# AlejandroSilvestri/os1

Hardware: AMD Instinct MI355X
Metric: frames/sec extract+match, 1920x1080 @ 2000 ORB feats (higher is better)
Workload: dtype u8

## Files before the change

### include/orbfe.h

```cpp
#ifndef ORBFE_H_
#define ORBFE_H_

#include <stddef.h>
#include <stdint.h>

#ifdef __cplusplus
extern "C" {
#endif

#define ORBFE_OK 0
#define ORBFE_ERR_INVALID (-1)
#define ORBFE_ERR_NO_DEVICE (-2)
#define ORBFE_ERR_HIP (-3)
#define ORBFE_ERR_TOO_SMALL (-4)
#define ORBFE_ERR_OVERFLOW (-5)
#define ORBFE_ERR_UNSUPPORTED (-6)

typedef struct OrbfeKeyPoint {
  float x, y;
  float size;
  float angle;
  float response;
  int32_t octave;
  int32_t class_id;
// ... 44 lines not shown

int orbfe_extract(orbfe_extractor* h, const uint8_t* gray, int rows, int cols, size_t stride_bytes,
                  OrbfeKeyPoint* kps, uint8_t* desc, int cap, int* n_out);

int orbfe_extract_batch(orbfe_extractor* h, int nframes, const uint8_t* const* gray, int in_device_memory,
                        int rows, int cols, size_t stride_bytes, OrbfeKeyPoint* kps, uint8_t* desc, int cap,
                        int* n_out);

int orbfe_extract_batch_submit(orbfe_extractor* h, int nframes, const uint8_t* const* gray, int in_device_memory,
                               int rows, int cols, size_t stride_bytes);
int orbfe_extract_batch_collect(orbfe_extractor* h, OrbfeKeyPoint* kps, uint8_t* desc, int cap, int* n_out);
int orbfe_extract_batch_wait(orbfe_extractor* h);

typedef struct orbfe_sfi_chain orbfe_sfi_chain;
int orbfe_sfi_chain_create(const orbfe_extractor* h, orbfe_sfi_chain** out);
void orbfe_sfi_chain_destroy(orbfe_sfi_chain* c);
int orbfe_sfi_chain_set_isolated(orbfe_sfi_chain* c, int isolated);
int orbfe_sfi_chain_restart(orbfe_sfi_chain* c);
int orbfe_extract_batch_submit_matched(orbfe_extractor* h, orbfe_sfi_chain* chain, int nframes, const uint8_t* const* gray,
                                       int in_device_memory, int rows, int cols, size_t stride_bytes, const float bounds[4],
                                       int window_size, float nnratio, int check_orientation);
int orbfe_extract_batch_collect_matched(orbfe_extractor* h, OrbfeKeyPoint* kps, uint8_t* desc, int cap, int* n_out,
                                        int32_t* matches12, int* nmatches);

int orbfe_extractor_set_camera(orbfe_extractor* h, int camera_mode, float fx, float fy, float cx, float cy, const float* dist,
                               int ndist);
int orbfe_extractor_undistort(orbfe_extractor* h, float* xy, int n);

int orbfe_extractor_set_camera_equidistant(orbfe_extractor* h, float fx, float fy, float cx, float cy);
int orbfe_extractor_undistort_verdict(orbfe_extractor* h, const float* xy, int n, float* out, uint8_t* undecided);
int orbfe_extractor_equidistant_stats(const orbfe_extractor* h, long long stats[3]);
int orbfe_extract_undistorted(orbfe_extractor* h, const uint8_t* gray, int rows, int cols, size_t stride_bytes, OrbfeKeyPoint* kps,
                              uint8_t* desc, int cap, int* n_out, float* xy_un);
int orbfe_extract_batch_collect_undistorted(orbfe_extractor* h, OrbfeKeyPoint* kps, uint8_t* desc, int cap, int* n_out, float* xy_un,
                                            int32_t* matches12, int* nmatches);

int orbfe_debug_level_size(const orbfe_extractor* h, int level, int* w, int* hgt);
int orbfe_debug_level_copy(orbfe_extractor* h, int frame, int level, uint8_t* out );
int orbfe_debug_candidates(orbfe_extractor* h, int frame, int level, int32_t* xys, int cap, int* n_out);
int orbfe_debug_stage_ms(const orbfe_extractor* h, float out[5]);
int orbfe_debug_kernel_ms(orbfe_extractor* h, double out_ms[5], long long* batches, long long* frames, int reset);
int orbfe_debug_set_profiling(orbfe_extractor* h, int enable);
int orbfe_debug_fast_stamps(orbfe_extractor* h, unsigned long long out[8], int reset);
int orbfe_debug_sfi_records(orbfe_extractor* h, int32_t* out, int cap_records, int* n_out, int reset);
int orbfe_debug_sincos(orbfe_extractor* h, const float* angle_deg, int n, float* cos_out, float* sin_out);

int orbfe_debug_quadtree(const int16_t* x, const int16_t* y, const uint8_t* score, int n, int min_x, int max_x,
                         int min_y, int max_y, int n_target, int32_t* out_idx, int cap, int* n_out);
int orbfe_debug_sincos_host_check(uint32_t lo_bits, uint32_t hi_bits, uint32_t step, long long* mismatches);
int orbfe_debug_logf(orbfe_matcher* m, const float* x, int n, float* out);
int orbfe_debug_logf_host_check(uint32_t lo_bits, uint32_t hi_bits, uint32_t step, long long* mismatches);

typedef struct orbfe_stream orbfe_stream;
int orbfe_stream_create(int nfeatures, float scaleFactor, int nlevels, int iniThFAST, int minThFAST, int device_id,
                        int batch, int depth, orbfe_stream** out);
void orbfe_stream_destroy(orbfe_stream* s);
int orbfe_stream_set_matching(orbfe_stream* s, const float bounds[4], int window_size, float nnratio,
                              int check_orientation);
int orbfe_stream_set_isolated_batches(orbfe_stream* s, int isolated);
int orbfe_stream_batches_in_flight(const orbfe_stream* s);
int orbfe_stream_pop_hold(orbfe_stream* s, const OrbfeKeyPoint** kps, const uint8_t** desc, const int** n_kps, const int32_t** matches12,
                          const int** nmatches, int* ticket);
int orbfe_stream_release(orbfe_stream* s, int ticket);
int orbfe_stream_set_input_format(orbfe_stream* s, int format, int gray_variant);
int orbfe_stream_set_blur_variant(orbfe_stream* s, int variant);
int orbfe_stream_set_vocabulary(orbfe_stream* s, orbfe_vocabulary* v, int levelsup);
int orbfe_stream_bow_raw(orbfe_stream* s, int frame, const uint32_t** leaf_node, const uint32_t** level_node, int* n);
int orbfe_stream_set_camera(orbfe_stream* s, int camera_mode, float fx, float fy, float cx, float cy, const float* dist, int ndist);
int orbfe_stream_set_camera_equidistant(orbfe_stream* s, float fx, float fy, float cx, float cy);
int orbfe_stream_equidistant_stats(orbfe_stream* s, long long stats[3]);
int orbfe_stream_xy_un(orbfe_stream* s, const float** xy_un);
int orbfe_stream_capacity(const orbfe_stream* s);
int orbfe_stream_set_queue_slots(orbfe_stream* s, int nslots);
int orbfe_stream_queue_slots(const orbfe_stream* s);
int orbfe_stream_push(orbfe_stream* s, const uint8_t* const* gray, int in_device_memory, int rows, int cols,
                      size_t stride_bytes);
int orbfe_stream_pop(orbfe_stream* s, const OrbfeKeyPoint** kps, const uint8_t** desc, const int** n_kps,
                     const int32_t** matches12, const int** nmatches);
int orbfe_stream_stats(orbfe_stream* s, double out[4], int reset);
int orbfe_stream_kernel_ms(orbfe_stream* s, double out_ms[5], long long* batches, long long* frames, int reset);


int orbfe_hamming(const uint8_t a[32], const uint8_t b[32]);

int orbfe_matcher_create(int device_id, orbfe_matcher** out);
void orbfe_matcher_destroy(orbfe_matcher* m);
int orbfe_matcher_device(const orbfe_matcher* m);
int orbfe_matcher_upload_async(orbfe_matcher* m, void* dst_device, const void* src_host, size_t bytes);
int orbfe_matcher_synchronize(orbfe_matcher* m);

int orbfe_search_for_initialization(orbfe_matcher* m, const OrbfeKeyPoint* kps1, const uint8_t* desc1, int n1,
                                    const OrbfeKeyPoint* kps2, const uint8_t* desc2, int n2,
                                    const float bounds[4], float* prev_xy, int32_t* matches12, int window_size,
                                    float nnratio, int check_orientation, int* nmatches);

int orbfe_search_for_initialization_batch(orbfe_matcher* m, int npairs, const OrbfeKeyPoint* const* kps1,
                                          const uint8_t* const* desc1, const int* n1,
                                          const OrbfeKeyPoint* const* kps2, const uint8_t* const* desc2,
                                          const int* n2, const float bounds[4], float* const* prev_xy,
                                          int32_t* const* matches12, int window_size, float nnratio,
                                          int check_orientation, int* nmatches);

#define ORBFE_MP_IN_VIEW 1u
#define ORBFE_MP_BAD 2u
#define ORBFE_MP_CANDIDATO 4u
#define ORBFE_MP_OBSERVED 8u
// ... 292 lines not shown
```

### os1_amd/csrc/orbfe_extractor.hip

```cpp
#include <hip/hip_runtime.h>
#include <unistd.h>
#include <sched.h>

#include <algorithm>
#include <cctype>
#include <chrono>
#include <cmath>
#include <cstdarg>
#include <cstdio>
#include <cstdlib>
#include <cstring>
#include <memory>
#include <mutex>
#include <string>
#include <thread>
#include <vector>

#include "../../include/orbfe.h"
#include "extract_plan.h"
#include "glibc_sincosf.h"
#include "host_pool.h"
#include "orbfe_internal.h"
#include "quadtree.h"

// ... 36 lines not shown

using namespace orbfe;

#define HIP_TRY(expr)                                                                        \
  do {                                                                                       \
    hipError_t e_ = (expr);                                                                  \
    if (e_ != hipSuccess) {                                                                  \
      set_err("%s failed: %s (%s:%d)", #expr, hipGetErrorString(e_), __FILE__, __LINE__);    \
      return ORBFE_ERR_HIP;                                                                  \
    }                                                                                        \
  } while (0)

namespace {
inline int cv_round_f(float v) { return (int)lrintf(v); }
inline int cv_floor_f(float v) { int i = (int)v; return i - (i > v); }
inline short sat_short(int v) { return (short)(v < -32768 ? -32768 : v > 32767 ? 32767 : v); }
inline long long align_up(long long v, long long a) { return (v + a - 1) / a * a; }
double now_ms() {
  return std::chrono::duration<double, std::milli>(std::chrono::steady_clock::now().time_since_epoch()).count();
}

template <class T>
struct DevBuf {
  T* p = nullptr;
  size_t n = 0;
  int ensure(size_t count) {
    if (count <= n) return ORBFE_OK;
    if (p) (void)hipFree(p);
    p = nullptr;
    n = 0;
    HIP_TRY(hipMalloc((void**)&p, count * sizeof(T)));
    n = count;
    return ORBFE_OK;
  }
  void release() { if (p) (void)hipFree(p); p = nullptr; n = 0; }
};
template <class T>
struct PinBuf {
  T* p = nullptr;
  size_t n = 0;
  int ensure(size_t count) {
    if (count <= n) return ORBFE_OK;
    if (p) (void)hipHostFree(p);
    p = nullptr;
    n = 0;
    HIP_TRY(hipHostMalloc((void**)&p, count * sizeof(T), hipHostMallocDefault));
    n = count;
    return ORBFE_OK;
  }
  void release() { if (p) (void)hipHostFree(p); p = nullptr; n = 0; }
};
}

struct orbfe_sfi_chain {
  int device = 0, n0cap = 0;
  DevBuf<SelKp> sel[2];
  DevBuf<float> angle[2];
  DevBuf<uint8_t> desc[2];
  DevBuf<float> xyUn[2];
  bool camera = false;
  DevBuf<uint32_t> count;
  hipEvent_t ready[2] = {};
  long long seq = 0;
  bool isolated = false;
  bool restart = false;
  orbfe_matcher* hostMatcher = nullptr;
  std::vector<OrbfeKeyPoint> hostPrevKps;
  std::vector<uint8_t> hostPrevDesc;
  bool hostPrevValid = false;
  std::vector<OrbfeKeyPoint> eqPrevKps;
  std::vector<uint8_t> eqPrevDesc;
  bool eqPrevValid = false, eqCarryStale = false;
  bool equi = false;
  float eqCam[4] = {0, 0, 0, 0};
  ~orbfe_sfi_chain() {
    (void)hipSetDevice(device);
    if (hostMatcher) orbfe_matcher_destroy(hostMatcher);
    for (int i = 0; i < 2; i++) { sel[i].release(); angle[i].release(); desc[i].release(); xyUn[i].release(); if (ready[i]) (void)hipEventDestroy(ready[i]); }
    count.release();
  }
};

struct UploadLane {
  std::mutex mu;
  hipStream_t stream = nullptr;
};
static UploadLane* upload_lane(int device) {
  static std::mutex mu;
  static UploadLane* lanes[64] = {};
  if (device < 0 || device >= 64) return nullptr;
  std::lock_guard<std::mutex> lk(mu);
  if (!lanes[device]) {
    UploadLane* l = new UploadLane;
    if (hipStreamCreateWithFlags(&l->stream, hipStreamNonBlocking) != hipSuccess) { delete l; return nullptr; }
    lanes[device] = l;
  }
  return lanes[device];
}

struct orbfe_extractor {
  int nfeatures, nlevels, iniTh, minTh, device;
  double scaleFactor;
  std::vector<float> sf, isf, sigma2, isigma2;
  std::vector<int> nfeat;
  hipStream_t stream = nullptr;
  hipEvent_t evUpload = nullptr;
  bool lastLocalCand = false, submitLocalCand = false;
  bool localLists = true;
  size_t candHostCap = 0;
  bool forceHostQt = false;
  bool submitHostSel = false;
  double hostSelMs = 0;
  orbfe_vocabulary* voc = nullptr;
  int vocLevelsup = 4;
  bool pendingBow = false;
  DevBuf<uint2> d_bow;
  PinBuf<uint2> h_bow;
  std::vector<std::vector<uint2>> bowKp;
  int kpPerFrameCap = 0;
  bool geomGpuQtOk = true;
  QtParams QP{};
  int selOff[kMaxLevels + 1] = {};
  int selPerFrame = 0;
  int n0cap = 0;
  DevBuf<uint16_t> d_own;
  hipEvent_t evQt[2] = {};

  int rows = 0, cols = 0, batchCap = 0;
  PyramidParams P{};
  DevBuf<uint8_t> d_tables, d_slab, d_in;
  DevBuf<ConeRange> d_coneTab, d_coneTailTab;
  ConeParams coneTail{};
  bool tailOk = false;
  int tailBase = 0, tailTile = 48;
  ConeParams cone{};
  bool coneOk = false;
  bool qtJump = true;
  int qtLdsBudget = 120 * 1024;
  int pollWaitUs = 0;
  bool zeroCopyOut = true;
  bool zeroCopyBatches = false;
  bool ingestKernel = true;
  int coneTile = 0;
  int coneMaxFrames = 2;
  DevBuf<FastCell> d_cells;
  DevBuf<uint8_t> d_zeros;
  DevBuf<uint32_t> d_cellCount, d_slots, d_cand;
  DevBuf<const uint8_t*> d_frame0;
  template <class T> struct View { T* p = nullptr; };
  DevBuf<uint8_t> d_outArena;
  PinBuf<uint8_t> h_outArena;
  size_t outArenaBytes = 0;
  View<uint32_t> d_levelStart, d_selCount, h_levelStart, h_selCount;
  View<SelKp> d_sel, h_sel;
  View<float> d_angle, h_angle;
  View<uint8_t> d_desc, h_desc;
  View<int32_t> d_m12, h_m12, d_nm, h_nm;
  bool camSet = false, camActive = false;
  CameraModel cam{};
  View<float> d_xyUn, h_xyUn;
  bool lastCam = false, submitCam = false;
  DevBuf<float> d_unTmp;
  PinBuf<float> h_unTmp;
  bool camEqui = false, submitEqui = false;
  EquidistantCamera camE{};
  float camF[4] = {0, 0, 0, 0};
  View<uint32_t> d_undec, h_undec;
  DevBuf<uint32_t> d_undecTmp;
  PinBuf<uint32_t> h_undecTmp;
  DevBuf<uint8_t> d_flagTmp;
  PinBuf<uint8_t> h_flagTmp;
  long long eqStats[3] = {0, 0, 0};
  std::vector<uint8_t> eqFrameChanged;
  std::vector<float> eqXy;
  std::vector<OrbfeKeyPoint> eqUn;
  std::vector<int32_t> eqRow;
  orbfe_sfi_chain* submitChain = nullptr;
  bool submitHasPred = false;
  DevBuf<uint16_t> d_sfiOrder;
  DevBuf<int> d_sfiOrderCount;
  DevBuf<uint32_t> d_sfiPool, d_sfiPcount;
  bool pendingMatched = false;
  DevBuf<float> d_f32tmp;
  bool profileKernels = false;
  PinBuf<const uint8_t*> h_frame0;
  PinBuf<uint32_t> h_cand;
  long long inPitch = 0;
  int inFormat = ORBFE_INPUT_GRAY8, grayVariant = ORBFE_GRAY_Q15;
  int gaussVariant = ORBFE_GAUSS_ED;
  long long grayPitch = 0;
  DevBuf<uint8_t> d_gray;
  bool inLinear = false;
  int lastFrames = 0;
  bool lastZeroCopy = false, submitZeroCopy = false;
  bool describe4 = true;
  float stageMs[5] = {0, 0, 0, 0, 0};
  hipEvent_t ev[6] = {};
  double kernMs[5] = {0, 0, 0, 0, 0};
  long long kernBatches = 0, kernFrames = 0;

  struct Worker {
    QuadTree qt;
    std::vector<int16_t> qx, qy;
    std::vector<uint8_t> qs;
    std::vector<int> qsel;
  };
  std::unique_ptr<HostPool> pool;
  int hostThreads = 1;
  std::vector<Worker> workers;

  ~orbfe_extractor() {
    (void)hipSetDevice(device);
    if (stream) (void)hipStreamSynchronize(stream);
    d_bow.release(); h_bow.release();
    d_tables.release(); d_coneTab.release(); d_coneTailTab.release(); d_slab.release(); d_in.release(); d_cellCount.release();
    d_sfiOrder.release(); d_sfiOrderCount.release(); d_sfiPool.release(); d_sfiPcount.release();
    d_cells.release(); d_zeros.release(); d_slots.release(); d_cand.release(); d_frame0.release(); d_gray.release(); d_outArena.release(); h_outArena.release();
    d_f32tmp.release(); d_unTmp.release(); h_unTmp.release();
    h_frame0.release(); h_cand.release();
    for (auto& e : ev) if (e) (void)hipEventDestroy(e);
    for (auto& e : evQt) if (e) (void)hipEventDestroy(e);
    d_own.release();
    if (evUpload) (void)hipEventDestroy(evUpload);
    if (stream) (void)hipStreamDestroy(stream);
  }

  bool hostSelect() const { return forceHostQt || !geomGpuQtOk; }

  int setGeometry(int r, int c) {
    if (r == rows && c == cols) return ORBFE_OK;
    if (c > 4095 || r > 4095) {
// ... 484 lines not shown
    if (matches12 && nmatches &&
        (rc = searchRowsOnHost(nframes, un, desc, cap, n_out, submitHasPred && ch.hostPrevValid ? &prev : nullptr, matches12, nmatches,
                               [](int) { return true; }, &nrows)))
      return rc;
    const int last = nframes - 1;
    ch.hostPrevKps.assign(un + (size_t)last * cap, un + (size_t)last * cap + n_out[last]);
    ch.hostPrevDesc.assign(desc + (size_t)last * cap * 32, desc + ((size_t)last * cap + n_out[last]) * 32);
    ch.hostPrevValid = !ch.isolated;
    return ORBFE_OK;
  }

  bool submitProfiled = false, fastTimed = false;
  std::vector<const uint8_t*> devAt;
  int pendingFrames = 0;
  double tSubmit0 = 0, tSubmit1 = 0;

  struct MatchSpec { orbfe_sfi_chain* chain; float bounds[4]; int window; float nnratio; int checkOri; };
  MatchSpec submitMs{};

  struct Route { bool small, hostSel, zeroCopy, kernelOut, localCand, prof; };

  int submit(int nframes, const uint8_t* const* gray, bool onDevice, int r, int c, size_t stride, const MatchSpec* ms = nullptr) {
    if (pendingFrames) { set_err("a submitted batch has not been collected yet"); return ORBFE_ERR_INVALID; }
    HIP_TRY(hipSetDevice(device));
    int rc;
    if ((rc = setGeometry(r, c))) return rc;
    if ((rc = setBatch(nframes, !onDevice, stride))) return rc;
    const double t0 = now_ms();
    hipStream_t st = stream;
    for (int f = 0; f < nframes; f++)
      if (!gray[f]) { set_err("frame %d is NULL", f); return ORBFE_ERR_INVALID; }
    Route R{};
    R.small = nframes <= coneMaxFrames;
    R.hostSel = hostSelect();
    R.zeroCopy = zeroCopyOut && R.small && !voc && !(ms && ms->chain) && !R.hostSel;
    R.kernelOut = zeroCopyBatches && !R.small && !R.hostSel;
    R.localCand = R.small && localLists && !R.hostSel;
    R.prof = profileKernels;
    submitZeroCopy = R.zeroCopy;
    submitLocalCand = R.localCand;
    submitHostSel = R.hostSel;
    submitCam = camActive;
    submitEqui = camEqui;
    if ((rc = framesToDevice(nframes, gray, onDevice, r, c, stride, st))) return rc;
    if ((rc = level0AndGray(nframes, gray, onDevice, r, c, stride, st))) return rc;
    if ((rc = front(nframes, R, st))) return rc;
    if ((rc = R.hostSel ? selectOnHost(nframes, st) : selectOnGpu(nframes, R, st))) return rc;
    if ((rc = describe(nframes, R, st))) return rc;
    if (camActive && (rc = undistortSlots(nframes, R, st))) return rc;
    pendingBow = false;
    if (voc && (rc = descendVocabulary(nframes, st))) return rc;
    pendingMatched = false;
    submitChain = nullptr;
    if (ms && ms->chain && (rc = matchChain(*ms, nframes, R, st))) return rc;
    if (!R.zeroCopy && !R.kernelOut) HIP_TRY(hipMemcpyAsync(h_outArena.p, d_outArena.p, outArenaBytes, hipMemcpyDeviceToHost, st));
    submitProfiled = R.prof;
    tSubmit0 = t0;
    tSubmit1 = now_ms();
    pendingFrames = nframes;
    return ORBFE_OK;
  }

  int framesToDevice(int nframes, const uint8_t* const* gray, bool onDevice, int r, int c, size_t stride, hipStream_t st) {
    int rc;
    const int rowBytes = c * inChannels();
    devAt.resize(nframes);
    bool pinned = !onDevice;
    std::vector<const uint8_t*>& mappedAt = devAt;
    if (!onDevice) {
      const size_t extent = stride * (size_t)(r - 1) + (size_t)rowBytes;
      const int ncheck = nframes <= coneMaxFrames ? nframes : 1;
      for (int f = 0; f < ncheck && pinned; f++) {
        void* dp = nullptr;
        void* dpEnd = nullptr;
        const bool ok = hipHostGetDevicePointer(&dp, const_cast<uint8_t*>(gray[f]), 0) == hipSuccess && dp &&
                        hipHostGetDevicePointer(&dpEnd, const_cast<uint8_t*>(gray[f]) + extent - 1, 0) == hipSuccess &&
                        (const uint8_t*)dpEnd - (const uint8_t*)dp == (ptrdiff_t)(extent - 1);
        if (!ok) { (void)hipGetLastError(); pinned = false; break; }
        mappedAt[f] = static_cast<const uint8_t*>(dp);
      }
    }
    if (!onDevice && !pinned) {
      if ((rc = uploadFrames(0, nframes, gray, stride, r, rowBytes, st, devAt.data()))) return rc;
    } else if (!onDevice && ingestKernel && nframes <= coneMaxFrames &&
               ((((uintptr_t)gray[0] | (uintptr_t)gray[nframes - 1] | (uintptr_t)stride | (uintptr_t)rowBytes) & 3) == 0)) {
      for (int f = 0; f < nframes; f++) {
        uint8_t* d = d_in.p + (size_t)inPitch * rows * f;
        launch_ingest(mappedAt[f], (long long)stride, d, inPitch, rowBytes, r, st);
        devAt[f] = d;
      }
      HIP_TRY(hipGetLastError());
    } else if (!onDevice) {
      UploadLane* lane = upload_lane(device);
      if (!lane) { set_err("cannot create the upload stream"); return ORBFE_ERR_HIP; }
      std::lock_guard<std::mutex> lk(lane->mu);
      if ((rc = uploadFrames(0, nframes, gray, stride, r, rowBytes, lane->stream, devAt.data()))) return rc;
      HIP_TRY(hipEventRecord(evUpload, lane->stream));
      HIP_TRY(hipStreamWaitEvent(st, evUpload, 0));
    }
    return ORBFE_OK;
  }

  int level0AndGray(int nframes, const uint8_t* const* gray, bool onDevice, int r, int c, size_t stride, hipStream_t st) {
    const int ch = inChannels();
    bool rawAligned = ((onDevice ? (long long)stride : inPitch) & 3) == 0;
    for (int f = 0; f < nframes; f++) {
// ... 137 lines not shown
    if (camEqui) {
      HIP_TRY(hipMemsetAsync(d_undec.p, 0, sizeof(uint32_t) * (1 + kUndecidedCap), st));
      EquidistantArgs E{};
      static_cast<UndistortSlots&>(E) = S;
      E.cam = camE; E.undecided = d_undec.p; E.flags = nullptr;
      launch_undistort_equidistant(E, st);
      if (zeroCopy || kernelOut) HIP_TRY(hipMemcpyAsync(h_undec.p, d_undec.p, sizeof(uint32_t) * (1 + kUndecidedCap), hipMemcpyDeviceToHost, st));
    } else {
      UndistortArgs U{};
      static_cast<UndistortSlots&>(U) = S;
      U.cam = cam;
      launch_undistort(U, st);
    }
    HIP_TRY(hipGetLastError());
    if (kernelOut) HIP_TRY(hipMemcpyAsync(h_xyUn.p, d_xyUn.p, 2 * sizeof(float) * (size_t)nslots, hipMemcpyDeviceToHost, st));
    return ORBFE_OK;
  }

  int descendVocabulary(int nframes, hipStream_t st) {
    const int nslots = nframes * selPerFrame;
    int rc;
    if ((rc = d_bow.ensure(nslots)) || (rc = h_bow.ensure(nslots))) return rc;
    if ((rc = bow_launch_descend(voc, d_desc.p, nslots, vocLevelsup, d_bow.p, st))) return rc;
    HIP_TRY(hipMemcpyAsync(h_bow.p, d_bow.p, sizeof(uint2) * nslots, hipMemcpyDeviceToHost, st));
    pendingBow = true;
    return ORBFE_OK;
  }

  int matchChain(const MatchSpec& spec, int nframes, const Route& R, hipStream_t st) {
    const MatchSpec* ms = &spec;
    const bool kernelOut = R.kernelOut;
    int rc;
    submitChain = ms->chain;
    submitMs = *ms;
    orbfe_sfi_chain& ch = *ms->chain;
    const bool otherModel = ch.equi != camEqui || (camEqui && memcmp(ch.eqCam, camF, sizeof camF));
    if (R.hostSel) {
      submitHasPred = !(ch.isolated || ch.restart || otherModel || ch.camera != camActive);
      ch.camera = camActive;
      ch.equi = camEqui;
      memcpy(ch.eqCam, camF, sizeof camF);
      ch.restart = false;
      pendingMatched = true;
      return ORBFE_OK;
    }
    if (otherModel) {
      if (ch.seq > 0) ch.restart = true;
      ch.eqPrevValid = ch.eqCarryStale = false;
    }
    ch.equi = camEqui;
    memcpy(ch.eqCam, camF, sizeof camF);
    submitHasPred = !(ch.seq == 0 || ch.isolated || ch.restart);
    if (ch.n0cap != n0cap || ch.device != device) { set_err("match chain belongs to a different extractor configuration"); return ORBFE_ERR_INVALID; }
    if ((rc = d_sfiOrder.ensure((size_t)batchCap * n0cap))) return rc;
    if ((rc = d_sfiOrderCount.ensure(batchCap))) return rc;
    if ((rc = d_sfiPool.ensure((size_t)batchCap * n0cap * n0cap))) return rc;
    if ((rc = d_sfiPcount.ensure((size_t)batchCap * n0cap))) return rc;
    SfiParams SP{};
    SP.sel = d_sel.p; SP.angle = d_angle.p; SP.desc = d_desc.p; SP.selCount = d_selCount.p;
    SP.selPerFrame = selPerFrame; SP.n0cap = n0cap; SP.frameBase = 0;
    const int prev = (int)((ch.seq + 1) & 1), cur = (int)(ch.seq & 1);
    SP.carrySel = ch.sel[prev].p; SP.carryAngle = ch.angle[prev].p; SP.carryDesc = ch.desc[prev].p;
    const bool iso = ch.isolated;
    if (camActive) {
      for (int i = 0; i < 2; i++)
        if ((rc = ch.xyUn[i].ensure(2 * (size_t)n0cap))) return rc;
    }
    if (ch.camera != camActive && ch.seq > 0) ch.restart = true;
    ch.camera = camActive;
    SP.xyUn = camActive ? d_xyUn.p : nullptr;
    SP.carryXyUn = camActive ? ch.xyUn[prev].p : nullptr;
    SP.carryCount = ch.count.p + ((ch.seq == 0 || iso || ch.restart) ? 2 : prev);
    ch.restart = false;
    SP.minX = ms->bounds[0]; SP.minY = ms->bounds[2];
    SP.invW = static_cast<float>(64) / static_cast<float>(ms->bounds[1] - ms->bounds[0]);
    SP.invH = static_cast<float>(48) / static_cast<float>(ms->bounds[3] - ms->bounds[2]);
    SP.window = (float)ms->window; SP.nnratio = ms->nnratio; SP.checkOri = ms->checkOri;
    SP.order = d_sfiOrder.p; SP.orderCount = d_sfiOrderCount.p; SP.pool = d_sfiPool.p; SP.pcount = d_sfiPcount.p;
    SP.matches12 = kernelOut ? h_m12.p : d_m12.p; SP.nmatches = kernelOut ? h_nm.p : d_nm.p;
    if (ch.seq > 0 && !iso) HIP_TRY(hipStreamWaitEvent(st, ch.ready[prev], 0));
    launch_sfi(SP, nframes, st);
    HIP_TRY(hipGetLastError());
    if (!iso) {
      launch_sfi_carry(SP, nframes - 1, ch.sel[cur].p, ch.angle[cur].p, ch.desc[cur].p, ch.count.p + cur, camActive ? ch.xyUn[cur].p : nullptr, st);
      HIP_TRY(hipGetLastError());
      HIP_TRY(hipEventRecord(ch.ready[cur], st));
    }
    ch.seq++;
    pendingMatched = true;
    return ORBFE_OK;
  }

  int waitOnly() {
    if (!pendingFrames) return ORBFE_OK;
    HIP_TRY(hipSetDevice(device));
    hipStream_t st = stream;
    if (pollWaitUs > 0) {
      hipError_t q;
      while ((q = hipStreamQuery(st)) == hipErrorNotReady) usleep((useconds_t)pollWaitUs);
      if (q != hipSuccess) HIP_TRY(q);
    }
    HIP_TRY(hipStreamSynchronize(st));
    return ORBFE_OK;
  }

  int collect(OrbfeKeyPoint* kps, uint8_t* desc, int cap, int* n_out, int32_t* matches12 = nullptr,
              int* nmatches = nullptr, float* xy_un = nullptr) {
    if (!pendingFrames) { set_err("no submitted batch to collect"); return ORBFE_ERR_INVALID; }
    HIP_TRY(hipSetDevice(device));
    const int nframes = pendingFrames;
    pendingFrames = 0;
    hipStream_t st = stream;
    const double t0 = tSubmit0, t1 = tSubmit1;
    const double t1b = now_ms();
    if (pollWaitUs > 0) {
      hipError_t q;
      while ((q = hipStreamQuery(st)) == hipErrorNotReady) usleep((useconds_t)pollWaitUs);
      if (q != hipSuccess) HIP_TRY(q);
    }
    HIP_TRY(hipStreamSynchronize(st));
    const double t2 = now_ms();
    {
      float ms = 0;
      if (fastTimed && hipEventElapsedTime(&ms, ev[1], ev[2]) == hipSuccess) kernMs[1] += ms;
      if (submitProfiled) {
        if (hipEventElapsedTime(&ms, ev[0], ev[1]) == hipSuccess) kernMs[0] += ms;
        if (hipEventElapsedTime(&ms, ev[2], ev[3]) == hipSuccess) kernMs[2] += ms;
        if (hipEventElapsedTime(&ms, ev[4], ev[5]) == hipSuccess) kernMs[3] += ms;
        if (!submitHostSel && hipEventElapsedTime(&ms, evQt[0], evQt[1]) == hipSuccess) kernMs[4] += ms;
      }
      if (fastTimed) {
        kernBatches++;
        kernFrames += nframes;
      }
    }
    int status = ORBFE_OK;
    if (submitEqui && (status = settleEquidistant(nframes))) return status;
    std::vector<float> xyOwn;
    if (pendingMatched && !xy_un && (submitEqui || (submitHostSel && submitCam))) {
      xyOwn.resize((size_t)nframes * cap * 2);
      xy_un = xyOwn.data();
    }
    if (pendingBow) bowKp.resize(nframes);
    else bowKp.clear();
    for (int f = 0; f < nframes; f++) {
      OrbfeKeyPoint* ko = kps + (size_t)f * cap;
      uint8_t* dout = desc + (size_t)f * cap * 32;
      if (pendingBow) bowKp[f].clear();
      int n = 0;
      for (int l = 0; l < nlevels; l++) {
        const int cnt = (int)h_selCount.p[(size_t)f * kMaxLevels + l];
        const size_t base = (size_t)f * selPerFrame + selOff[l];
        const float scale = sf[l];
        const float size = (float)(int)(31 * sf[l]);
        for (int i = 0; i < cnt; i++) {
          if (n >= cap) { n++; continue; }
          const SelKp s = h_sel.p[base + i];
          OrbfeKeyPoint kp;
          kp.x = (float)(s.xy & 0xffff);
          kp.y = (float)(s.xy >> 16);
          if (l != 0) { kp.x *= scale; kp.y *= scale; }
          kp.size = size;
          kp.angle = h_angle.p[base + i];
          kp.response = (float)(s.lf >> 24);
          kp.octave = l;
          kp.class_id = -1;
          ko[n] = kp;
          memcpy(dout + (size_t)n * 32, h_desc.p + (base + i) * 32, 32);
          if (pendingBow) bowKp[f].push_back(h_bow.p[base + i]);
          if (xy_un) {
            float* u = xy_un + ((size_t)f * cap + n) * 2;
            u[0] = submitCam ? h_xyUn.p[2 * (base + i)] : kp.x;
            u[1] = submitCam ? h_xyUn.p[2 * (base + i) + 1] : kp.y;
// ... 493 lines not shown
  if (!h->camEqui) { set_err("the extractor has no equidistant camera (orbfe_extractor_set_camera_equidistant)"); return ORBFE_ERR_INVALID; }
  if (h->pendingFrames) { set_err("a submitted batch has not been collected yet"); return ORBFE_ERR_INVALID; }
  HIP_TRY(hipSetDevice(h->device));
  return h->equidistantPoints(const_cast<float*>(xy), n, out, undecided);
}

int orbfe_extractor_equidistant_stats(const orbfe_extractor* h, long long stats[3]) {
  if (!h || !stats) { set_err("NULL argument"); return ORBFE_ERR_INVALID; }
  for (int i = 0; i < 3; i++) stats[i] = h->eqStats[i];
  return ORBFE_OK;
}

int orbfe_extractor_undistort(orbfe_extractor* h, float* xy, int n) {
  if (!h || n < 0 || (n && !xy)) { set_err("bad argument"); return ORBFE_ERR_INVALID; }
  if (!h->camSet) { set_err("the extractor has no camera (orbfe_extractor_set_camera)"); return ORBFE_ERR_INVALID; }
  if (h->pendingFrames) { set_err("a submitted batch has not been collected yet"); return ORBFE_ERR_INVALID; }
  HIP_TRY(hipSetDevice(h->device));
  return h->undistortPoints(xy, n);
}

int orbfe_extract_batch_submit(orbfe_extractor* h, int nframes, const uint8_t* const* gray, int in_device_memory,
                               int rows, int cols, size_t stride_bytes) {
  if (!h || !gray || nframes <= 0 || rows <= 0 || cols <= 0 || stride_bytes < (size_t)cols * h->inChannels()) {
    set_err("invalid arguments");
    return ORBFE_ERR_INVALID;
  }
  return h->submit(nframes, gray, in_device_memory != 0, rows, cols, stride_bytes);
}

int orbfe_extract_batch_wait(orbfe_extractor* h) {
  if (!h) { set_err("invalid arguments"); return ORBFE_ERR_INVALID; }
  return h->waitOnly();
}

int orbfe_extract_batch_collect(orbfe_extractor* h, OrbfeKeyPoint* kps, uint8_t* desc, int cap, int* n_out) {
  if (!h || !kps || !desc || !n_out || cap <= 0) { set_err("invalid arguments"); return ORBFE_ERR_INVALID; }
  return h->collect(kps, desc, cap, n_out);
}

int orbfe_extract_batch_collect_undistorted(orbfe_extractor* h, OrbfeKeyPoint* kps, uint8_t* desc, int cap, int* n_out, float* xy_un,
                                            int32_t* matches12, int* nmatches) {
  if (!h || !kps || !desc || !n_out || !xy_un || cap <= 0 || (!matches12) != (!nmatches)) { set_err("invalid arguments"); return ORBFE_ERR_INVALID; }
  return h->collect(kps, desc, cap, n_out, matches12, nmatches, xy_un);
}

int orbfe_sfi_chain_create(const orbfe_extractor* h, orbfe_sfi_chain** out) {
  if (!h || !out) { set_err("NULL argument"); return ORBFE_ERR_INVALID; }
  *out = nullptr;
  HIP_TRY(hipSetDevice(h->device));
  orbfe_sfi_chain* c = new orbfe_sfi_chain();
  c->device = h->device;
  c->n0cap = h->n0cap;
  int rc = ORBFE_OK;
  for (int i = 0; i < 2 && rc == ORBFE_OK; i++) {
    if ((rc = c->sel[i].ensure(c->n0cap))) break;
    if ((rc = c->angle[i].ensure(c->n0cap))) break;
    if ((rc = c->desc[i].ensure((size_t)c->n0cap * 32))) break;
    if (hipEventCreateWithFlags(&c->ready[i], hipEventDisableTiming) != hipSuccess) { set_err("hipEventCreate failed"); rc = ORBFE_ERR_HIP; }
  }
  if (rc == ORBFE_OK) rc = c->count.ensure(4);
  if (rc == ORBFE_OK) {
    const uint32_t init[4] = {0xffffffffu, 0xffffffffu, 0xffffffffu, 0xffffffffu};
    if (hipMemcpy(c->count.p, init, sizeof init, hipMemcpyHostToDevice) != hipSuccess) { set_err("hipMemcpy failed"); rc = ORBFE_ERR_HIP; }
  }
  if (rc != ORBFE_OK) { delete c; return rc; }
  *out = c;
  return ORBFE_OK;
}

void orbfe_sfi_chain_destroy(orbfe_sfi_chain* c) { delete c; }

int orbfe_sfi_chain_set_isolated(orbfe_sfi_chain* c, int isolated) {
  if (!c) { set_err("chain is NULL"); return ORBFE_ERR_INVALID; }
  if (c->isolated != (isolated != 0)) {
    c->seq = 0;
    c->hostPrevValid = false;
  }
  c->isolated = isolated != 0;
  return ORBFE_OK;
}

int orbfe_sfi_chain_restart(orbfe_sfi_chain* c) {
  if (!c) { set_err("chain is NULL"); return ORBFE_ERR_INVALID; }
  c->restart = true;
  return ORBFE_OK;
}

int orbfe_extract_batch_submit_matched(orbfe_extractor* h, orbfe_sfi_chain* chain, int nframes, const uint8_t* const* gray,
                                       int in_device_memory, int rows, int cols, size_t stride_bytes, const float bounds[4],
                                       int window_size, float nnratio, int check_orientation) {
  if (!h || !chain || !gray || !bounds || nframes <= 0 || rows <= 0 || cols <= 0 || stride_bytes < (size_t)cols * h->inChannels() || window_size <= 0) {
    set_err("invalid arguments");
    return ORBFE_ERR_INVALID;
  }
  if (!(bounds[1] > bounds[0] && bounds[3] > bounds[2])) { set_err("empty image bounds"); return ORBFE_ERR_INVALID; }
  orbfe_extractor::MatchSpec ms;
  ms.chain = chain;
  memcpy(ms.bounds, bounds, sizeof ms.bounds);
  ms.window = window_size;
  ms.nnratio = nnratio;
  ms.checkOri = check_orientation;
  return h->submit(nframes, gray, in_device_memory != 0, rows, cols, stride_bytes, &ms);
}

int orbfe_extract_batch_collect_matched(orbfe_extractor* h, OrbfeKeyPoint* kps, uint8_t* desc, int cap, int* n_out,
                                        int32_t* matches12, int* nmatches) {
  if (!h || !kps || !desc || !n_out || !matches12 || !nmatches || cap <= 0) { set_err("invalid arguments"); return ORBFE_ERR_INVALID; }
  return h->collect(kps, desc, cap, n_out, matches12, nmatches);
}

int orbfe_extract(orbfe_extractor* h, const uint8_t* gray, int rows, int cols, size_t stride_bytes, OrbfeKeyPoint* kps,
                  uint8_t* desc, int cap, int* n_out) {
  if (!n_out) { set_err("n_out is NULL"); return ORBFE_ERR_INVALID; }
  *n_out = 0;
  if (!gray || rows == 0 || cols == 0) return ORBFE_OK;
  const uint8_t* frames[1] = {gray};
  return orbfe_extract_batch(h, 1, frames, 0, rows, cols, stride_bytes, kps, desc, cap, n_out);
}

int orbfe_extract_undistorted(orbfe_extractor* h, const uint8_t* gray, int rows, int cols, size_t stride_bytes, OrbfeKeyPoint* kps,
                              uint8_t* desc, int cap, int* n_out, float* xy_un) {
  if (!n_out || !xy_un) { set_err("n_out or xy_un is NULL"); return ORBFE_ERR_INVALID; }
  *n_out = 0;
  if (!gray || rows == 0 || cols == 0) return ORBFE_OK;
  const uint8_t* frames[1] = {gray};
  return extract_batch_impl(h, 1, frames, 0, rows, cols, stride_bytes, kps, desc, cap, n_out, xy_un);
}

int orbfe_debug_level_size(const orbfe_extractor* h, int level, int* w, int* hgt) {
// ... 119 lines not shown
```

### os1_amd/csrc/orbfe_stream.cpp

```cpp
#include <pthread.h>

#include <algorithm>
#include <chrono>
#include <condition_variable>
#include <cstdio>
#include <cstdlib>
#include <cstring>
#include <deque>
#include <mutex>
#include <string>
#include <thread>
#include <vector>

#include "../../include/orbfe.h"

namespace orbfe {
void set_err(const char* fmt, ...);
}
int orbfe_concurrent_streams(orbfe_extractor* const* hs, int n);
using orbfe::set_err;

namespace {
struct Slot {
  std::vector<const uint8_t*> frames;
// ... 161 lines not shown
        if (s.camera) {
          s.xyUn.resize((size_t)batch * cap * 2);
          const bool m = s.window > 0;
          s.status = orbfe_extract_batch_collect_undistorted(ext[e], s.kps.data(), s.desc.data(), cap, s.n.data(), s.xyUn.data(),
                                                             m ? s.m12.data() : nullptr, m ? s.nm.data() : nullptr);
        } else if (s.window > 0)
          s.status = orbfe_extract_batch_collect_matched(ext[e], s.kps.data(), s.desc.data(), cap, s.n.data(), s.m12.data(),
                                                         s.nm.data());
        else
          s.status = orbfe_extract_batch_collect(ext[e], s.kps.data(), s.desc.data(), cap, s.n.data());
        if (s.status == ORBFE_OK && bow) {
          s.bowLeaf.resize((size_t)batch * cap);
          s.bowNode.resize((size_t)batch * cap);
          for (int f = 0; f < batch && s.status == ORBFE_OK; f++) {
            int nb = 0;
            s.status = orbfe_extract_bow_raw(ext[e], f, s.bowLeaf.data() + (size_t)f * cap, s.bowNode.data() + (size_t)f * cap, cap, &nb);
          }
        }
        {
          std::lock_guard<std::mutex> lk(mu);
          busyCollect += nowMs() - ta;
        }
        if (s.status != ORBFE_OK) s.err = orbfe_last_error();
      }
      if (s.status == ORBFE_OK) {
        s.prevN = isolated ? -1 : lastN;
        if (s.prevN >= 0) { s.prevKps = lastKps; s.prevDesc = lastDesc; if (s.camera) s.prevXyUn = lastXyUn; }
        if (s.window <= 0) {
          std::fill(s.nm.begin(), s.nm.end(), 0);
          std::fill(s.m12.begin(), s.m12.end(), -1);
        } else if (s.frame0OnHost && s.prevN >= 0) {
          s.status = matchFrame0(s);
          if (s.status != ORBFE_OK) s.err = orbfe_last_error();
        }
        lastN = s.n[batch - 1];
        lastKps.assign(s.kps.begin() + (size_t)(batch - 1) * cap, s.kps.begin() + (size_t)(batch - 1) * cap + lastN);
        lastDesc.assign(s.desc.begin() + (size_t)(batch - 1) * cap * 32, s.desc.begin() + ((size_t)(batch - 1) * cap + lastN) * 32);
        if (s.camera) lastXyUn.assign(s.xyUn.begin() + (size_t)(batch - 1) * cap * 2, s.xyUn.begin() + ((size_t)(batch - 1) * cap + lastN) * 2);
      }
      {
        std::lock_guard<std::mutex> lk(mu);
        nBatches++;
        s.done = true;
      }
      cv.notify_all();
    }
  }
};

extern "C" {

int orbfe_stream_create(int nfeatures, float scaleFactor, int nlevels, int iniThFAST, int minThFAST, int device_id,
                        int batch, int depth, orbfe_stream** out) {
  if (!out || batch < 1 || depth < 1 || depth > 8) { set_err("invalid stream parameters"); return ORBFE_ERR_INVALID; }
  *out = nullptr;
  orbfe_stream* s = new orbfe_stream();
  s->batch = batch;
  s->depth = depth;
  s->device = device_id;
  const int nhandles = depth;
  for (int d = 0; d < nhandles; d++) {
    orbfe_extractor* h = nullptr;
    int rc = orbfe_extractor_create(nfeatures, scaleFactor, nlevels, iniThFAST, minThFAST, device_id, &h);
    if (rc == ORBFE_OK && !getenv("ORBFE_POLL_WAIT_US")) rc = orbfe_extractor_set_wait_mode(h, 50);
    if (rc != ORBFE_OK) {
      for (auto* e : s->ext) orbfe_extractor_destroy(e);
      delete s;
      return rc;
    }
    s->ext.push_back(h);
  }
  {
    int rc = orbfe_sfi_chain_create(s->ext[0], &s->chain);
    if (rc != ORBFE_OK) {
      for (auto* e : s->ext) orbfe_extractor_destroy(e);
      delete s;
      return rc;
    }
  }
  s->inFlight = depth;
  if (depth > 1) {
    const int k = orbfe_concurrent_streams(s->ext.data(), depth);
    if (k < 0) {
      for (auto* e : s->ext) orbfe_extractor_destroy(e);
      orbfe_sfi_chain_destroy(s->chain);
      delete s;
      return k;
    }
    s->inFlight = k;
    while ((int)s->ext.size() > k) {
      orbfe_extractor_destroy(s->ext.back());
      s->ext.pop_back();
    }
    static bool said = false;
    if (k < depth && !said && !getenv("ORBFE_QUIET")) {
      said = true;
      const char* q = getenv("GPU_MAX_HW_QUEUES");
      fprintf(stderr, "liborbfe: orbfe_stream_create(depth = %d): only %d of the runner's streams run side by side in this process (GPU_MAX_HW_QUEUES=%s), "
                      "so %d batches are kept in flight; export GPU_MAX_HW_QUEUES=8 before the process starts for the last 3 %%\n",
              depth, k, q ? q : "unset: 4", k);
    }
  }
  s->cap = orbfe_extractor_max_keypoints(s->ext[0]);
  s->growSlots(depth + 4);
  s->tExtract = std::thread([s] { pthread_setname_np(pthread_self(), "orbfe-runner"); s->extractLoop(); });
  *out = s;
  return ORBFE_OK;
// ... 310 lines not shown
```

### os1_amd/csrc/orbfe_stream_multi.cpp

```cpp
#include <pthread.h>

#include <cstring>
#include <memory>
#include <string>
#include <thread>
#include <vector>

#include "../../include/orbfe.h"
#include "inorder_gate.h"

namespace orbfe {
void set_err(const char* fmt, ...);
}
using orbfe::set_err;
extern "C" int orbfe_stream_capacity_for(const orbfe_stream* s, int rows, int cols);
extern "C" int orbfe_stream_grow_capacity(orbfe_stream* s, int need);
extern "C" const float* orbfe_stream_held_xy_un(orbfe_stream* s, int ticket);

struct orbfe_stream_multi {
  int ndev = 0, batch = 0;
  int cap = 0;
  std::vector<int> devices;
  std::vector<orbfe_stream*> sub;
  std::vector<orbfe_matcher*> matcher;
// ... 80 lines not shown
          std::unique_lock<std::mutex> lk(mu);
          cv.wait(lk, [&] { return stop || tailOf(k - 1).seq == k - 1; });
          if (tailOf(k - 1).seq != k - 1) return;
          if (matching) prev = tailOf(k - 1);
          tailRead[(size_t)((k - 1) % ndev)] = k - 1;
        }
        cv.notify_all();
        if (matching && r.status == ORBFE_OK && prev.n >= 0 && !noPred_k && (r.xyUn != nullptr) == (prev.n == 0 || !prev.xyUn.empty())) {
          int32_t* m12 = const_cast<int32_t*>(r.m12);
          int* nm = const_cast<int*>(r.nm);
          prevxy.resize((size_t)(prev.n > 0 ? prev.n : 1) * 2);
          for (int j = 0; j < prev.n; j++) { prevxy[2 * j] = prev.kps[j].x; prevxy[2 * j + 1] = prev.kps[j].y; }
          row.assign((size_t)(prev.n > 0 ? prev.n : 1), -1);
          int nmatch = 0;
          const OrbfeKeyPoint* k2 = r.kps;
          if (r.xyUn) {
            cur.assign(r.kps, r.kps + r.n[0]);
            for (int j = 0; j < r.n[0]; j++) { cur[(size_t)j].x = r.xyUn[2 * j]; cur[(size_t)j].y = r.xyUn[2 * j + 1]; }
            for (int j = 0; j < prev.n; j++) { prev.kps[(size_t)j].x = prevxy[2 * j] = prev.xyUn[2 * (size_t)j]; prev.kps[(size_t)j].y = prevxy[2 * j + 1] = prev.xyUn[2 * (size_t)j + 1]; }
            k2 = cur.data();
          }
          const int rc = orbfe_search_for_initialization(matcher[d], prev.kps.data(), prev.desc.data(), prev.n, k2, r.desc, r.n[0], bounds_k,
                                                         prevxy.data(), row.data(), window_k, nnratio_k, checkOri_k, &nmatch);
          if (rc != ORBFE_OK) {
            r.status = rc;
            r.err = orbfe_last_error();
          } else {
            const int m = prev.n < stride ? prev.n : stride;
            memcpy(m12, row.data(), sizeof(int32_t) * (size_t)m);
            for (int i = m; i < stride; i++) m12[i] = -1;
            nm[0] = nmatch;
          }
        }
      }
      doneOf(k) = r;
      gate->publish(k);
    }
  }
};

static void release_held_batch(orbfe_stream_multi* s) {
  if (s->heldSeq >= 0) {
    const orbfe_stream_multi::Done& r = s->doneOf(s->heldSeq);
    if (r.ticket >= 0) (void)orbfe_stream_release(s->sub[(size_t)(s->heldSeq % s->ndev)], r.ticket);
    s->heldSeq = -1;
  }
  s->gate->release_held();
}

extern "C" {

int orbfe_stream_multi_create(int nfeatures, float scaleFactor, int nlevels, int iniThFAST, int minThFAST, const int* device_ids,
                              int n_devices, int batch, int depth, orbfe_stream_multi** out) {
  if (!out || !device_ids || n_devices < 1 || n_devices > 64 || batch < 1 || depth < 1 || depth > 8) {
    set_err("invalid multi-device stream parameters");
    return ORBFE_ERR_INVALID;
  }
  *out = nullptr;
  std::unique_ptr<orbfe_stream_multi> s(new orbfe_stream_multi());
  s->ndev = n_devices;
  s->batch = batch;
  s->devices.assign(device_ids, device_ids + n_devices);
  s->done.resize((size_t)n_devices * orbfe_stream_multi::kRing);
  s->tail.resize((size_t)n_devices * 2);
  s->tailRead.assign((size_t)n_devices, -1);
  s->gate.reset(new orbfe::InOrderGate(n_devices));
  int rc = ORBFE_OK;
  std::string err;
  for (int d = 0; d < n_devices && rc == ORBFE_OK; d++) {
    std::thread helper([&, d] {
      (void)orbfe_bind_thread_to_device(device_ids[d]);
      orbfe_stream* sub = nullptr;
      int r = orbfe_stream_create(nfeatures, scaleFactor, nlevels, iniThFAST, minThFAST, device_ids[d], batch, depth, &sub);
      if (r == ORBFE_OK) {
        s->sub.push_back(sub);
        r = orbfe_stream_set_isolated_batches(sub, 1);
      }
      if (r == ORBFE_OK) {
        orbfe_matcher* m = nullptr;
        r = orbfe_matcher_create(device_ids[d], &m);
        if (r == ORBFE_OK) s->matcher.push_back(m);
      }
      if (r != ORBFE_OK) err = orbfe_last_error();
      rc = r;
    });
    helper.join();
  }
  if (rc != ORBFE_OK) {
    set_err("%s", err.c_str());
    for (auto* q : s->sub) orbfe_stream_destroy(q);
    for (auto* m : s->matcher) orbfe_matcher_destroy(m);
    return rc;
  }
  s->cap = orbfe_stream_capacity(s->sub[0]);
  orbfe_stream_multi* p = s.release();
  for (int d = 0; d < n_devices; d++)
    p->finisher.emplace_back([p, d] {
      pthread_setname_np(pthread_self(), "orbfe-finish");
      (void)orbfe_bind_thread_to_device(p->devices[(size_t)d]);
      p->finish(d);
    });
  *out = p;
  return ORBFE_OK;
}

void orbfe_stream_multi_destroy(orbfe_stream_multi* s) {
  if (!s) return;
// ... 173 lines not shown
```

Measured before the change: 89720.

## Widen match-chain carry buffers to a depth-sized ring and launch carry before matching

Measured after the change: 89320. About the same (-0.4%).

```diff
diff --git a/include/orbfe.h b/include/orbfe.h
--- a/include/orbfe.h
+++ b/include/orbfe.h
@@ -120,6 +120,7 @@
 int orbfe_debug_logf_host_check(uint32_t lo_bits, uint32_t hi_bits, uint32_t step, long long* mismatches);
 
 typedef struct orbfe_stream orbfe_stream;
+#define ORBFE_STREAM_MAX_DEPTH 8
 int orbfe_stream_create(int nfeatures, float scaleFactor, int nlevels, int iniThFAST, int minThFAST, int device_id,
                         int batch, int depth, orbfe_stream** out);
 void orbfe_stream_destroy(orbfe_stream* s);
diff --git a/os1_amd/csrc/orbfe_extractor.hip b/os1_amd/csrc/orbfe_extractor.hip
--- a/os1_amd/csrc/orbfe_extractor.hip
+++ b/os1_amd/csrc/orbfe_extractor.hip
@@ -112,15 +112,17 @@
 };
 }
 
+constexpr int kSfiRing = ORBFE_STREAM_MAX_DEPTH + 1;
 struct orbfe_sfi_chain {
   int device = 0, n0cap = 0;
-  DevBuf<SelKp> sel[2];
-  DevBuf<float> angle[2];
-  DevBuf<uint8_t> desc[2];
-  DevBuf<float> xyUn[2];
+  DevBuf<SelKp> sel[kSfiRing];
+  DevBuf<float> angle[kSfiRing];
+  DevBuf<uint8_t> desc[kSfiRing];
+  DevBuf<float> xyUn[kSfiRing];
   bool camera = false;
   DevBuf<uint32_t> count;
-  hipEvent_t ready[2] = {};
+  hipEvent_t ready[kSfiRing] = {};
+  bool uncollected[kSfiRing] = {};
   long long seq = 0;
   bool isolated = false;
   bool restart = false;
@@ -136,7 +138,7 @@
   ~orbfe_sfi_chain() {
     (void)hipSetDevice(device);
     if (hostMatcher) orbfe_matcher_destroy(hostMatcher);
-    for (int i = 0; i < 2; i++) { sel[i].release(); angle[i].release(); desc[i].release(); xyUn[i].release(); if (ready[i]) (void)hipEventDestroy(ready[i]); }
+    for (int i = 0; i < kSfiRing; i++) { sel[i].release(); angle[i].release(); desc[i].release(); xyUn[i].release(); if (ready[i]) (void)hipEventDestroy(ready[i]); }
     count.release();
   }
 };
@@ -237,6 +239,7 @@
   std::vector<int32_t> eqRow;
   orbfe_sfi_chain* submitChain = nullptr;
   bool submitHasPred = false;
+  int submitRing = -1;
   DevBuf<uint16_t> d_sfiOrder;
   DevBuf<int> d_sfiOrderCount;
   DevBuf<uint32_t> d_sfiPool, d_sfiPcount;
@@ -827,6 +830,7 @@
     if (voc && (rc = descendVocabulary(nframes, st))) return rc;
     pendingMatched = false;
     submitChain = nullptr;
+    submitRing = -1;
     if (ms && ms->chain && (rc = matchChain(*ms, nframes, R, st))) return rc;
     if (!R.zeroCopy && !R.kernelOut) HIP_TRY(hipMemcpyAsync(h_outArena.p, d_outArena.p, outArenaBytes, hipMemcpyDeviceToHost, st));
     submitProfiled = R.prof;
@@ -1070,6 +1074,12 @@
     memcpy(ch.eqCam, camF, sizeof camF);
     submitHasPred = !(ch.seq == 0 || ch.isolated || ch.restart);
     if (ch.n0cap != n0cap || ch.device != device) { set_err("match chain belongs to a different extractor configuration"); return ORBFE_ERR_INVALID; }
+    const int prev = (int)((ch.seq + kSfiRing - 1) % kSfiRing), cur = (int)(ch.seq % kSfiRing);
+    const bool iso = ch.isolated;
+    if (!iso && ch.uncollected[(cur + 1) % kSfiRing]) {
+      set_err("match chain: more than %d batches submitted and not collected", kSfiRing - 1);
+      return ORBFE_ERR_INVALID;
+    }
     if ((rc = d_sfiOrder.ensure((size_t)batchCap * n0cap))) return rc;
     if ((rc = d_sfiOrderCount.ensure(batchCap))) return rc;
     if ((rc = d_sfiPool.ensure((size_t)batchCap * n0cap * n0cap))) return rc;
@@ -1077,18 +1087,17 @@
     SfiParams SP{};
     SP.sel = d_sel.p; SP.angle = d_angle.p; SP.desc = d_desc.p; SP.selCount = d_selCount.p;
     SP.selPerFrame = selPerFrame; SP.n0cap = n0cap; SP.frameBase = 0;
-    const int prev = (int)((ch.seq + 1) & 1), cur = (int)(ch.seq & 1);
     SP.carrySel = ch.sel[prev].p; SP.carryAngle = ch.angle[prev].p; SP.carryDesc = ch.desc[prev].p;
-    const bool iso = ch.isolated;
     if (camActive) {
-      for (int i = 0; i < 2; i++)
+      for (int i = 0; i < kSfiRing; i++)
         if ((rc = ch.xyUn[i].ensure(2 * (size_t)n0cap))) return rc;
     }
     if (ch.camera != camActive && ch.seq > 0) ch.restart = true;
     ch.camera = camActive;
     SP.xyUn = camActive ? d_xyUn.p : nullptr;
     SP.carryXyUn = camActive ? ch.xyUn[prev].p : nullptr;
-    SP.carryCount = ch.count.p + ((ch.seq == 0 || iso || ch.restart) ? 2 : prev);
+    const bool readsCarry = !(ch.seq == 0 || iso || ch.restart);
+    SP.carryCount = ch.count.p + (readsCarry ? prev : kSfiRing);
     ch.restart = false;
     SP.minX = ms->bounds[0]; SP.minY = ms->bounds[2];
     SP.invW = static_cast<float>(64) / static_cast<float>(ms->bounds[1] - ms->bounds[0]);
@@ -1096,14 +1105,16 @@
     SP.window = (float)ms->window; SP.nnratio = ms->nnratio; SP.checkOri = ms->checkOri;
     SP.order = d_sfiOrder.p; SP.orderCount = d_sfiOrderCount.p; SP.pool = d_sfiPool.p; SP.pcount = d_sfiPcount.p;
     SP.matches12 = kernelOut ? h_m12.p : d_m12.p; SP.nmatches = kernelOut ? h_nm.p : d_nm.p;
-    if (ch.seq > 0 && !iso) HIP_TRY(hipStreamWaitEvent(st, ch.ready[prev], 0));
-    launch_sfi(SP, nframes, st);
-    HIP_TRY(hipGetLastError());
     if (!iso) {
       launch_sfi_carry(SP, nframes - 1, ch.sel[cur].p, ch.angle[cur].p, ch.desc[cur].p, ch.count.p + cur, camActive ? ch.xyUn[cur].p : nullptr, st);
       HIP_TRY(hipGetLastError());
       HIP_TRY(hipEventRecord(ch.ready[cur], st));
-    }
+      ch.uncollected[cur] = true;
+      submitRing = cur;
+    }
+    if (readsCarry) HIP_TRY(hipStreamWaitEvent(st, ch.ready[prev], 0));
+    launch_sfi(SP, nframes, st);
+    HIP_TRY(hipGetLastError());
     ch.seq++;
     pendingMatched = true;
     return ORBFE_OK;
@@ -1137,6 +1148,10 @@
       if (q != hipSuccess) HIP_TRY(q);
     }
     HIP_TRY(hipStreamSynchronize(st));
+    if (submitRing >= 0) {
+      submitChain->uncollected[submitRing] = false;
+      submitRing = -1;
+    }
     const double t2 = now_ms();
     {
       float ms = 0;
@@ -1736,15 +1751,16 @@
   c->device = h->device;
   c->n0cap = h->n0cap;
   int rc = ORBFE_OK;
-  for (int i = 0; i < 2 && rc == ORBFE_OK; i++) {
+  for (int i = 0; i < kSfiRing && rc == ORBFE_OK; i++) {
     if ((rc = c->sel[i].ensure(c->n0cap))) break;
     if ((rc = c->angle[i].ensure(c->n0cap))) break;
     if ((rc = c->desc[i].ensure((size_t)c->n0cap * 32))) break;
     if (hipEventCreateWithFlags(&c->ready[i], hipEventDisableTiming) != hipSuccess) { set_err("hipEventCreate failed"); rc = ORBFE_ERR_HIP; }
   }
-  if (rc == ORBFE_OK) rc = c->count.ensure(4);
+  if (rc == ORBFE_OK) rc = c->count.ensure(kSfiRing + 1);
   if (rc == ORBFE_OK) {
-    const uint32_t init[4] = {0xffffffffu, 0xffffffffu, 0xffffffffu, 0xffffffffu};
+    uint32_t init[kSfiRing + 1];
+    for (uint32_t& v : init) v = 0xffffffffu;
     if (hipMemcpy(c->count.p, init, sizeof init, hipMemcpyHostToDevice) != hipSuccess) { set_err("hipMemcpy failed"); rc = ORBFE_ERR_HIP; }
   }
   if (rc != ORBFE_OK) { delete c; return rc; }
@@ -1759,6 +1775,8 @@
   if (c->isolated != (isolated != 0)) {
     c->seq = 0;
     c->hostPrevValid = false;
+    c->eqPrevValid = c->eqCarryStale = false;
+    for (bool& u : c->uncollected) u = false;
   }
   c->isolated = isolated != 0;
   return ORBFE_OK;
diff --git a/os1_amd/csrc/orbfe_stream.cpp b/os1_amd/csrc/orbfe_stream.cpp
--- a/os1_amd/csrc/orbfe_stream.cpp
+++ b/os1_amd/csrc/orbfe_stream.cpp
@@ -237,7 +237,7 @@
 
 int orbfe_stream_create(int nfeatures, float scaleFactor, int nlevels, int iniThFAST, int minThFAST, int device_id,
                         int batch, int depth, orbfe_stream** out) {
-  if (!out || batch < 1 || depth < 1 || depth > 8) { set_err("invalid stream parameters"); return ORBFE_ERR_INVALID; }
+  if (!out || batch < 1 || depth < 1 || depth > ORBFE_STREAM_MAX_DEPTH) { set_err("invalid stream parameters"); return ORBFE_ERR_INVALID; }
   *out = nullptr;
   orbfe_stream* s = new orbfe_stream();
   s->batch = batch;
diff --git a/os1_amd/csrc/orbfe_stream_multi.cpp b/os1_amd/csrc/orbfe_stream_multi.cpp
--- a/os1_amd/csrc/orbfe_stream_multi.cpp
+++ b/os1_amd/csrc/orbfe_stream_multi.cpp
@@ -156,7 +156,7 @@
 
 int orbfe_stream_multi_create(int nfeatures, float scaleFactor, int nlevels, int iniThFAST, int minThFAST, const int* device_ids,
                               int n_devices, int batch, int depth, orbfe_stream_multi** out) {
-  if (!out || !device_ids || n_devices < 1 || n_devices > 64 || batch < 1 || depth < 1 || depth > 8) {
+  if (!out || !device_ids || n_devices < 1 || n_devices > 64 || batch < 1 || depth < 1 || depth > ORBFE_STREAM_MAX_DEPTH) {
     set_err("invalid multi-device stream parameters");
     return ORBFE_ERR_INVALID;
   }
```
